# rbuler/multimodal-isic

Measured on AMD Instinct MI355X. Metric: bags/sec (train step) @ 64x224x224 patches/bag, higher is better.
Workload: dtype bf16; 1 GPU; ISIC-shaped attention-MIL: 256 bags x 64x224x224 patches + 128-d radiomics, ResNet-18 encoder, bf16 (BASELINE.json configs[1]); patches_per_bag=64, patch=3x224x224, radiomics_dim=128, parallelism=dp1

## Files before the change

### include/isic_hip.h

```cpp
#ifndef ISIC_HIP_H
#define ISIC_HIP_H

#include <stddef.h>
#include <stdint.h>

#ifdef __cplusplus
extern "C" {
#endif

#define ISIC_OK 0
#define ISIC_ERR_BAD_ARG (-1)
#define ISIC_ERR_UNSUPPORTED (-2)
#define ISIC_ERR_WORKSPACE (-3)
#define ISIC_ERR_LAUNCH (-4)

#define ISIC_ACT_NONE 0
#define ISIC_ACT_RELU 1
#define ISIC_ACT_TANH 2

int isic_abi_version(void);
const char* isic_target_arch(void);

int isic_gemm_f32(int transA, int transB, int M, int N, int K, const float* A, int lda, const float* B, int ldb,
                  float* C, int ldc, const float* bias, int act, float beta, void* stream);
// ... 231 lines not shown
                                   const float* rstd, int N, int H, int W, int C, int Ho, int Wo, const float* scale,
                                   const float* shift, double* dgamma, double* dbeta, void* stream);
int isic_bn_bwd_apply_pooled_bf16(const uint8_t* argmax, const uint16_t* dy_pooled, const uint16_t* x, const float* mean,
                                  const float* rstd, const float* gamma, const double* dgamma, const double* dbeta, int N,
                                  int H, int W, int C, int Ho, int Wo, const float* scale, const float* shift,
                                  uint16_t* dx, float* dgamma_f32, float* dbeta_f32, void* stream);
int isic_avgpool_fwd_bf16(const uint16_t* x, float* y, int N, int HW, int C, void* stream);
int isic_avgpool_bwd_bf16(const float* dy, uint16_t* dx, int N, int HW, int C, void* stream);
int isic_add_bf16(uint16_t* a, const uint16_t* b, int64_t n, void* stream);

int isic_gemm_f16(const uint16_t* A, const uint16_t* W, const float* bias, const uint16_t* residual, uint16_t* C,
                  int M, int N, int K, int act, int residual_rows, void* stream);
int isic_gemm_f16_stats(const uint16_t* A, const uint16_t* W, const float* bias, const uint16_t* residual, uint16_t* C,
                        float* row_stats, int M, int N, int K, int act, int residual_rows, void* stream);
int isic_gemm_f16_ln(const uint16_t* X, const uint16_t* Wg, const float* bias_b, const float* ln_c, const float* ln_stats,
                     int ln_parts, uint16_t* C, int M, int N, int K, int act, float eps, void* stream);
int isic_row_stats_f16(const uint16_t* x, float* stats, int64_t M, int N, float eps, void* stream);
int isic_vit_patchify_f16(const float* images_nchw, uint16_t* rows, int N, int C, int H, int W, int P, void* stream);
int isic_layernorm_f16(const uint16_t* x, const float* gamma, const float* beta, uint16_t* y, float* y_f32, int64_t M,
                       int N, float eps, void* stream);
int isic_attention_f16(const uint16_t* qkv, uint16_t* out, int n_images, int tokens, int heads, int head_dim,
                       void* stream);

#ifdef __cplusplus
}
#endif

#include "isic_hip_mxfp8.h"
#include "isic_hip_vit_train.h"
#include "isic_hip_convmae.h"
#include "isic_hip_convmae_train.h"
#include "isic_hip_mae.h"
#include "isic_hip_augment.h"

#endif
```

### multimodal-isic_amd/csrc/conv_wgrad.hip

```cpp
#include "common.h"

namespace {

struct WgradArgs {
  const unsigned short* x;
  const unsigned short* dy;
  float* dw;
  size_t split_stride;
  const int2* tab;
  int N, Hin, Win, Cin, Hout, Wout, Cout, Kh, Kw, stride, pad;
  int M;
  int ktiles;
  int ktiles_per_split;
  int co_tiles, ci_tiles;
};

__global__ void wgrad_table_kernel(int2* __restrict__ tab, int M, int Hout, int Wout, int Hin, int Win, int Cin,
                                   int stride, int pad) {
  const int m = blockIdx.x * blockDim.x + threadIdx.x;
  if (m >= M) return;
  const int hw = Hout * Wout;
  const int n = m / hw, r = m - n * hw;
  const int ho = r / Wout, wo = r - ho * Wout;
  int2 e;
// ... 168 lines not shown
  if (e < elems && g == 0) dw[e] += v;
}

struct WgradPlan {
  bool big;
  int tiles, splits, ktiles, ktiles_per_split;
  size_t table_bytes, partial_bytes, elems;
};

WgradPlan wgrad_plan(int N, int Cin, int Hout, int Wout, int Cout, int Kh, int Kw) {
  WgradPlan p;
  const int M = N * Hout * Wout;
  p.big = (Cin % 128 == 0) && (Cout % 128 == 0);
  const int tc = p.big ? 128 : 64, bkp = p.big ? 64 : 128;
  p.ktiles = ceil_div(M, bkp);
  p.tiles = (Cout / tc) * (Cin / tc) * Kh * Kw;
  int splits = ceil_div(1280, p.tiles);
  if (splits > ceil_div(p.ktiles, 8)) splits = ceil_div(p.ktiles, 8);
  if (splits < 1) splits = 1;
  if (splits > 4096) splits = 4096;
  p.ktiles_per_split = ceil_div(p.ktiles, splits);
  p.splits = ceil_div(p.ktiles, p.ktiles_per_split);
  p.table_bytes = ((size_t)M * sizeof(int2) + 255) / 256 * 256;
  p.elems = (size_t)Cout * Kh * Kw * Cin;
  p.partial_bytes = (size_t)p.splits * p.elems * sizeof(float);
  return p;
}

}

size_t isic_wgrad_c64_workspace_bytes(int N, int H, int W);
int isic_wgrad_c64_launch(const uint16_t* x, const uint16_t* dy, float* dw, int N, int H, int W, void* workspace,
                          hipStream_t stream);

size_t isic_wgrad_c128b_workspace_bytes(int N, int H, int W, int Cin, int Cout);
int isic_wgrad_c128b_launch(const uint16_t* x, const uint16_t* dy, float* dw, int N, int H, int W, int Cin, int Cout,
                            void* workspace, hipStream_t stream);

size_t isic_wgrad_s2_workspace_bytes(int N, int Hi, int Wi, int Cin, int Cout);
int isic_wgrad_s2_launch(const uint16_t* x, const uint16_t* dy, float* dw, int N, int Hi, int Wi, int Cin, int Cout,
                         void* workspace, hipStream_t stream);

namespace {
int conv2d_wgrad_dispatch(const uint16_t* x, const uint16_t* dy, float* dw, int N, int Hin, int Win, int Cin,
                          int Hout, int Wout, int Cout, int Kh, int Kw, int stride, int pad, void* workspace,
                          size_t workspace_bytes, int variant, void* stream);
}

extern "C" {

size_t isic_conv2d_wgrad_workspace_bytes(int N, int Cin, int Hout, int Wout, int Cout, int Kh, int Kw) {
  if (N <= 0 || Cin <= 0 || Hout <= 0 || Wout <= 0 || Cout <= 0 || Kh <= 0 || Kw <= 0) return 0;
  const WgradPlan p = wgrad_plan(N, Cin, Hout, Wout, Cout, Kh, Kw);
  size_t need = p.table_bytes + p.partial_bytes + 256;
  if (Cin == 64 && Cout == 64 && Kh == 3 && Kw == 3) {
    const size_t c64 = isic_wgrad_c64_workspace_bytes(N, Hout, Wout);
    if (c64 > need) need = c64;
  }
  if (Cin % 128 == 0 && Cout % 64 == 0 && Kh == 3 && Kw == 3) {
    const size_t c128b = isic_wgrad_c128b_workspace_bytes(N, Hout, Wout, Cin, Cout);
    if (c128b > need) need = c128b;
  }
  if (Cin % 64 == 0 && Cout % 128 == 0 && Kh == 3 && Kw == 3) {
    const size_t s2 = isic_wgrad_s2_workspace_bytes(N, 2 * Hout, 2 * Wout, Cin, Cout);
    if (s2 > need) need = s2;
  }
  return need;
}

int isic_conv2d_wgrad_bf16(const uint16_t* x, const uint16_t* dy, float* dw, int N, int Hin, int Win, int Cin,
                           int Hout, int Wout, int Cout, int Kh, int Kw, int stride, int pad, void* workspace,
                           size_t workspace_bytes, void* stream) {
  return conv2d_wgrad_dispatch(x, dy, dw, N, Hin, Win, Cin, Hout, Wout, Cout, Kh, Kw, stride, pad, workspace, workspace_bytes,
                               0, stream);
}

int isic_test_conv2d_wgrad_variant_bf16(const uint16_t* x, const uint16_t* dy, float* dw, int N, int Hin, int Win, int Cin,
                                        int Hout, int Wout, int Cout, int Kh, int Kw, int stride, int pad, void* workspace,
                                        size_t workspace_bytes, int variant, void* stream) {
  return conv2d_wgrad_dispatch(x, dy, dw, N, Hin, Win, Cin, Hout, Wout, Cout, Kh, Kw, stride, pad, workspace, workspace_bytes,
                               variant, stream);
}

}

namespace {

int conv2d_wgrad_dispatch(const uint16_t* x, const uint16_t* dy, float* dw, int N, int Hin, int Win, int Cin,
                          int Hout, int Wout, int Cout, int Kh, int Kw, int stride, int pad, void* workspace,
                          size_t workspace_bytes, int variant, void* stream) {
  ISIC_CHECK_ARG(x && dy && dw && workspace);
  ISIC_CHECK_ARG(N > 0 && Hin > 0 && Win > 0 && Hout > 0 && Wout > 0 && Kh > 0 && Kw > 0 && stride > 0 && pad >= 0);
  ISIC_CHECK_ARG((reinterpret_cast<uintptr_t>(workspace) & 255) == 0 && (reinterpret_cast<uintptr_t>(dw) & 15) == 0);
  ISIC_CHECK_ARG((variant & ~(16 | 32)) == 0);
  if (Cin % 64 != 0 || Cout % 64 != 0) return ISIC_ERR_UNSUPPORTED;
  const int64_t M64 = (int64_t)N * Hout * Wout;
  if (M64 > 0x7FFFFFFFLL / 2 || (int64_t)N * Hin * Win * Cin > 0x7FFFFFFFLL || Hout >= 32768 || Wout >= 32768)
    return ISIC_ERR_UNSUPPORTED;
  if (Cin == 64 && Cout == 64 && Kh == 3 && Kw == 3 && stride == 1 && pad == 1 && Hin == Hout && Win == Wout) {
    const size_t need = isic_wgrad_c64_workspace_bytes(N, Hin, Win);
    if (need != 0) {
      if (workspace_bytes < need) return ISIC_ERR_WORKSPACE;
      const int rc = isic_wgrad_c64_launch(x, dy, dw, N, Hin, Win, workspace, as_stream(stream));
      return rc != ISIC_OK ? rc : isic_launch_status();
    }
  }
  if (Cin % 128 == 0 && Cout % 64 == 0 && Kh == 3 && Kw == 3 && stride == 1 && pad == 1 && Hin == Hout && Win == Wout &&
// ... 46 lines not shown
```

### multimodal-isic_amd/csrc/conv_wgrad_c64.hip

```cpp

#include "common.h"

namespace {

constexpr int WT_H = 4, WT_W = 32;
constexpr int XP = 48;
constexpr int X_ROWS = WT_H + 2;
constexpr int X_BYTES = X_ROWS * XP * 128;
constexpr int DY_BYTES = WT_H * WT_W * 128;
constexpr int STAGE = X_BYTES + DY_BYTES;
constexpr int NSTAGE = 3;
constexpr int SCRATCH = NSTAGE * STAGE;
constexpr int LDS_TOTAL = SCRATCH + 1024;
constexpr int NDMA = 12;
constexpr int DW_ELEMS = 64 * 9 * 64;

struct WC64Args {
  const unsigned short* x;
  const unsigned short* dy;
  float* partial;
  int N, H, W, tiles_y, tiles_x, total_tiles, tiles_per_block;
};

__device__ __attribute__((aligned(256))) unsigned char g_wc64_zeros[2048];

__device__ __forceinline__ void glds16(const void* gsrc, unsigned lds_dst) {
  unsigned keep;
  asm volatile("s_mov_b32 %0, m0\n\ts_mov_b32 m0, %2\n\ts_nop 0\n\tglobal_load_lds_dwordx4 %1, off\n\ts_mov_b32 m0, %0"
               : "=&s"(keep) : "v"(gsrc), "s"(lds_dst) : "memory");
}

#ifdef WC64_STAMPS
__device__ unsigned long long g_wc64_stamps[256 * 64 * 4];
#define WC64_STAMP(kk, k) do { if (threadIdx.x == 512 && blockIdx.x < 256 && (kk) < 64) g_wc64_stamps[(blockIdx.x * 64 + (kk)) * 4 + (k)] = clock64(); } while (0)
#else
#define WC64_STAMP(kk, k) do { } while (0)
#endif

__global__ __launch_bounds__(768) void wgrad_c64_kernel(WC64Args a) {
  extern __shared__ __attribute__((aligned(16))) unsigned char smem[];
  typedef __attribute__((address_space(3))) s16x4* lds_s16x4;
  const unsigned lds0 = (unsigned)(size_t)(__attribute__((address_space(3))) unsigned char*)smem;
  const int tid = threadIdx.x, lane = tid & 63, wave12 = __builtin_amdgcn_readfirstlane(tid >> 6);
  const int t_begin = blockIdx.x * a.tiles_per_block;
  const int ntl = min(a.total_tiles - t_begin, a.tiles_per_block);

  if (wave12 >= 8) {
    const int p = wave12 - 8;
    const int tiles_img = a.tiles_y * a.tiles_x;
    struct Tile { int n, y0, x0; };
    auto advance = [&](Tile& tl) {
      tl.x0 += WT_W;
      if (tl.x0 >= a.W) {
        tl.x0 = 0; tl.y0 += WT_H;
        if (tl.y0 >= a.H) { tl.y0 = 0; tl.n += 1; }
      }
    };
    Tile ahead;
    {
      const int n = t_begin / tiles_img, rem = t_begin - n * tiles_img;
      const int ty = rem / a.tiles_x;
      ahead.n = n; ahead.y0 = ty * WT_H; ahead.x0 = (rem - ty * a.tiles_x) * WT_W;
    }
    const int r8 = lane >> 3, slot = lane & 7;
    const unsigned lane_e = (unsigned)(r8 * 128 + ((((slot >> 1) ^ ((r8 >> 1) & 1)) << 5) | ((slot & 1) << 4)));
    const unsigned lane_p = lane_e ^ (unsigned)((p & 1) << 6);
    const long long W128 = (long long)a.W * 128;
    const unsigned long long zeros = (unsigned long long)g_wc64_zeros;
    auto issue_tile = [&](const Tile& tl, int stage, bool live) {
      const long long org = ((long long)tl.n * a.H + tl.y0) * a.W + tl.x0;
      const unsigned long long xrow = (unsigned long long)a.x + (unsigned long long)((org - a.W - 1 + 8 * p) * 128);
      const unsigned long long yrow = (unsigned long long)a.dy + (unsigned long long)((org + 8 * p) * 128);
      const unsigned long long erow = (unsigned long long)a.x + (unsigned long long)((org + (long long)(2 * p - 1) * a.W + 31) * 128);
      const bool okx = (unsigned)(tl.x0 - 1 + 8 * p + r8) < (unsigned)a.W;
      const bool oky = (unsigned)(tl.x0 + 8 * p + r8) < (unsigned)a.W;
      const bool oke = (unsigned)(tl.x0 + 31 + r8) < (unsigned)a.W;
      const unsigned sbase = lds0 + (unsigned)stage * STAGE;
#pragma unroll
      for (int j = 0; j < NDMA; ++j) {
        unsigned long long rowaddr;
        bool okc, row_ok, real = live;
        unsigned lanev, dst;
        if (j < 6) {
          rowaddr = xrow + (unsigned long long)(j * W128);
          row_ok = (unsigned)(tl.y0 - 1 + j) < (unsigned)a.H; okc = okx; lanev = lane_p;
          dst = (unsigned)((j * XP + 8 * p) * 128);
        } else if (j < 10) {
          rowaddr = yrow + (unsigned long long)((j - 6) * W128);
          row_ok = (unsigned)(tl.y0 + j - 6) < (unsigned)a.H; okc = oky; lanev = lane_p;
          dst = (unsigned)(X_BYTES + ((j - 6) * 4 + p) * 1024);
        } else {
          const int pr = 2 * p + (j - 10);
          rowaddr = erow + (unsigned long long)((j - 10) * W128);
          row_ok = (unsigned)(tl.y0 - 1 + pr) < (unsigned)a.H; okc = oke; lanev = lane_e;
          real = real && pr < X_ROWS;
          dst = (unsigned)((pr * XP + 32) * 128);
        }
        const bool ok = okc && row_ok && real;
        const unsigned lo = ok ? (unsigned)rowaddr : (unsigned)zeros, hi = ok ? (unsigned)(rowaddr >> 32) : (unsigned)(zeros >> 32);
        const unsigned long long src = (((unsigned long long)hi << 32) | lo) + lanev;
        glds16(reinterpret_cast<const void*>(src), real ? sbase + dst : lds0 + SCRATCH);
      }
    };
    issue_tile(ahead, 0, true);
    advance(ahead);
    issue_tile(ahead, 1, ntl > 1);
    advance(ahead);
    for (int kk = 0; kk < ntl; ++kk) {
      WC64_STAMP(kk, 0);
      asm volatile("s_waitcnt vmcnt(%0)" ::"n"(NDMA) : "memory");
      WC64_STAMP(kk, 3);
      __builtin_amdgcn_s_barrier();
      WC64_STAMP(kk, 1);
      issue_tile(ahead, (kk + 2) % NSTAGE, kk + 2 < ntl);
      advance(ahead);
      WC64_STAMP(kk, 2);
    }
    return;
  }

  const int wave = wave12 & 3, half = wave12 >> 2;
  const int fg = lane >> 4, fi = lane & 15, fq = fi >> 2, fp = fi & 3;
  unsigned xaddr[3][2];
#pragma unroll
  for (int kw = 0; kw < 3; ++kw)
#pragma unroll
    for (int h = 0; h < 2; ++h) {
      const int px = 8 * fg + fq + kw + 4 * h;
      const int key = ((px >> 1) & 1) | (((px >> 3) & 1) << 1);
      xaddr[kw][h] = (unsigned)(px * 128 + ((wave ^ key) << 5) + fp * 8);
    }
  unsigned yaddr[2];
  {
    const int key = ((fq >> 1) & 1) | ((fg & 1) << 1);
#pragma unroll
    for (int c2 = 0; c2 < 2; ++c2) yaddr[c2] = (unsigned)(X_BYTES + (8 * fg + fq) * 128 + (((2 * half + c2) ^ key) << 5) + fp * 8);
// ... 73 lines not shown
    f32x4 t = red[0][q];
#pragma unroll
    for (int g = 1; g < 16; ++g) t += red[g][q];
    f32x4* out = reinterpret_cast<f32x4*>(dw) + e4;
    *out = *out + t;
  }
}

int wc64_blocks(int N, int H, int W, int* tiles_per_block) {
  const int cus = isic_cu_count();
  const int64_t total = (int64_t)N * ceil_div(H, WT_H) * ceil_div(W, WT_W);
  const int tpb = (int)ceil_div64(total, cus);
  if (tiles_per_block) *tiles_per_block = tpb;
  return (int)ceil_div64(total, tpb);
}

}

size_t isic_wgrad_c64_workspace_bytes(int N, int H, int W) {
  if ((int64_t)N * ceil_div(H, WT_H) * ceil_div(W, WT_W) > 0x7FFFFFFFLL) return 0;
  return (size_t)wc64_blocks(N, H, W, nullptr) * DW_ELEMS * sizeof(float);
}

int isic_wgrad_c64_launch(const uint16_t* x, const uint16_t* dy, float* dw, int N, int H, int W, void* workspace,
                          hipStream_t stream) {
  WC64Args a;
  a.x = x; a.dy = dy; a.partial = reinterpret_cast<float*>(workspace);
  a.N = N; a.H = H; a.W = W;
  a.tiles_y = ceil_div(H, WT_H); a.tiles_x = ceil_div(W, WT_W);
  a.total_tiles = N * a.tiles_y * a.tiles_x;
  const int grid = wc64_blocks(N, H, W, &a.tiles_per_block);
  static IsicPerDeviceOnce once;
  if (isic_once_per_device(once, [] {
        return hipFuncSetAttribute(reinterpret_cast<const void*>(wgrad_c64_kernel), hipFuncAttributeMaxDynamicSharedMemorySize,
                                  LDS_TOTAL);
      }) != hipSuccess)
    return ISIC_ERR_LAUNCH;
  hipLaunchKernelGGL(wgrad_c64_kernel, dim3(grid), dim3(768), LDS_TOTAL, stream, a);
  hipLaunchKernelGGL(wgrad_c64_reduce_kernel, dim3(DW_ELEMS / 64), dim3(256), 0, stream, a.partial, dw, grid);
  return ISIC_OK;
}
```

### multimodal-isic_amd/isic_hip/build.py

```python
from __future__ import annotations

import os
import shutil
import subprocess
import sys
from concurrent.futures import ThreadPoolExecutor

HERE = os.path.dirname(os.path.abspath(__file__))
PKG = os.path.dirname(HERE)
CSRC = os.path.join(PKG, "csrc")
OBJ = os.path.join(CSRC, "build")
LIB = os.path.join(HERE, "libisic_hip.so")
ARCH = "gfx950"
FLAGS = ["-O3", "-fPIC", "-std=c++17", f"--offload-arch={ARCH}", "-Wall", "-Wno-unused-function",
         "-Wno-unused-variable"]


def _hipcc():
    for c in (os.environ.get("HIPCC"), shutil.which("hipcc"), "/opt/rocm/bin/hipcc"):
        if c and os.path.exists(c):
            return c
    raise RuntimeError("hipcc not found: libisic_hip.so cannot be built")


def sources():
    return sorted(os.path.join(CSRC, f) for f in os.listdir(CSRC) if f.endswith(".hip"))


def _stale(target, deps):
    if not os.path.exists(target):
        return True
    t = os.path.getmtime(target)
    return any(os.path.getmtime(d) > t for d in deps)


def build(force=False, verbose=True, jobs=None):
    hipcc = _hipcc()
    os.makedirs(OBJ, exist_ok=True)
    headers = [os.path.join(CSRC, f) for f in os.listdir(CSRC) if f.endswith(".h")]
    headers += [os.path.join(os.path.dirname(PKG), "include", h)
                for h in ("isic_hip.h", "isic_hip_mxfp8.h", "isic_hip_vit_train.h", "isic_hip_convmae.h",
                          "isic_hip_convmae_train.h", "isic_hip_mae.h", "isic_hip_augment.h")]
    todo, objs = [], []
    for src in sources():
        obj = os.path.join(OBJ, os.path.basename(src)[:-4] + ".o")
        objs.append(obj)
        if force or _stale(obj, [src] + headers):
            todo.append((src, obj))

    def compile_one(so):
        src, obj = so
        cmd = [hipcc] + FLAGS + ["-c", src, "-o", obj]
        r = subprocess.run(cmd, capture_output=True, text=True)
        if r.returncode != 0:
            raise RuntimeError(f"hipcc failed for {src}:\n{r.stdout}\n{r.stderr}")
        if verbose and r.stderr.strip():
            sys.stderr.write(r.stderr)
        return obj

    if todo:
        if verbose:
            print(f"[isic_hip] compiling {len(todo)} HIP source(s) for {ARCH}", flush=True)
        with ThreadPoolExecutor(max_workers=jobs or min(8, os.cpu_count() or 4)) as ex:
            list(ex.map(compile_one, todo))
    if force or todo or _stale(LIB, objs):
        cmd = [hipcc, "-shared", "-fPIC", f"--offload-arch={ARCH}", "-o", LIB] + objs
        r = subprocess.run(cmd, capture_output=True, text=True)
        if r.returncode != 0:
            raise RuntimeError(f"link failed:\n{r.stdout}\n{r.stderr}")
        if verbose:
            print(f"[isic_hip] linked {LIB}", flush=True)
    return LIB


if __name__ == "__main__":
# ... 2 lines not shown
```

### multimodal-isic_amd/isic_hip/encoder.py

```python
from __future__ import annotations

import os

import torch
import torch.nn as nn

from .lib import ERR_UNSUPPORTED, IsicHipError, call

LAYERS = ((64, 1), (128, 2), (256, 2), (512, 2))
BN_EPS, BN_MOMENTUM = 1e-5, 0.1
STAT_SLOTS = 256
STEM_STAT_SLOTS = 1024
_BF16 = torch.bfloat16


def _empty(shape, like, dtype=_BF16):
    return torch.empty(shape, device=like.device, dtype=dtype)


class _ConvSpec:
    __slots__ = ("name", "cin", "cout", "k", "stride", "pad")

    def __init__(self, name, cin, cout, k, stride, pad):
        self.name, self.cin, self.cout, self.k, self.stride, self.pad = name, cin, cout, k, stride, pad
# ... 21 lines not shown
            self._register(name + ".bias", nn.Parameter(torch.zeros(c)))
            self._register(name + ".running_mean", torch.zeros(c), buffer=True)
            self._register(name + ".running_var", torch.ones(c), buffer=True)
            self._register(name + ".num_batches_tracked", torch.zeros((), dtype=torch.long), buffer=True)

        conv("conv1", in_ch, 64, 7, 2, 3)
        bn("bn1", 64)
        inp = 64
        self.blocks = []
        for li, (planes, stride) in enumerate(self.layers_cfg, start=1):
            for b in range(2):
                pre = f"layer{li}.{b}"
                st = stride if b == 0 else 1
                conv(f"{pre}.conv1", inp, planes, 3, st, 1)
                bn(f"{pre}.bn1", planes)
                conv(f"{pre}.conv2", planes, planes, 3, 1, 1)
                bn(f"{pre}.bn2", planes)
                ds = st != 1 or inp != planes
                if ds:
                    conv(f"{pre}.downsample.0", inp, planes, 1, st, 0)
                    bn(f"{pre}.downsample.1", planes)
                self.blocks.append((pre, ds))
                inp = planes
        self._wcache = {}
        self._wgrad_ws = None
        self._zeros = None
        self._zeros_used = 0
        self._side = None
        self.wgrad_stream = False
        self.fuse_bn_backward = False
        self.mask_identity_gradient = True
        self.pair_downsample_gradient = True
        self.fold_shortcut_norm = True
        self._tape_fused = False
        self.grad_ready_hook = None

    def _register(self, dotted, tensor, buffer=False):
        parts = dotted.split(".")
        mod = self
        for p in parts[:-1]:
            if not hasattr(mod, p):
                mod.add_module(p, nn.Module())
            mod = getattr(mod, p)
        if buffer:
            mod.register_buffer(parts[-1], tensor)
        else:
            mod.register_parameter(parts[-1], tensor)

    def _get(self, dotted):
        mod = self
        for p in dotted.split("."):
            mod = getattr(mod, p)
        return mod

    def _apply(self, fn, *a, **k):
        out = super()._apply(fn, *a, **k)
        for name in self.specs:
            p = self._get(name + ".weight")
            if not p.data.is_contiguous(memory_format=torch.channels_last):
                p.data = p.data.contiguous(memory_format=torch.channels_last)
        self._wcache = {}
        return out

    def prepare_weights(self):
        for name, sp in self.specs.items():
            p = self._get(name + ".weight")
            if not p.is_cuda:
# ... 191 lines not shown
                call("isic_bn_stats_bf16", c, rows, C, acc[0], acc[1])
            mean = torch.empty(C, device=dev, dtype=torch.float32)
            rstd = torch.empty(C, device=dev, dtype=torch.float32)
            call("isic_bn_finalize", acc[0], acc[1], slots, rows, C, gamma.data, beta.data, BN_EPS, BN_MOMENTUM, scale,
                 shift, mean, rstd, self._get(name + ".running_mean"), self._get(name + ".running_var"))
        else:
            call("isic_bn_eval_affine", gamma.data, beta.data, self._get(name + ".running_mean"),
                 self._get(name + ".running_var"), BN_EPS, C, scale, shift)
        return mean, rstd, scale, shift

    def _bn_bwd(self, dy, c, y, st, name, relu, want_residual, mask_from_x=False):
        mean, rstd, scale, shift = st[:4]
        mask = st[4] if len(st) > 4 else None
        N, H, W, C = c.shape
        rows = N * H * W
        gamma, beta = self._get(name + ".weight"), self._get(name + ".bias")
        acc = self._zeros64((2, C), c.device)
        if mask is not None and relu and not mask_from_x:
            call("isic_bn_bwd_reduce_mask_bf16", dy, c, mask, mean, rstd, rows, C, acc[0], acc[1])
            dx = _empty(c.shape, c)
            dres = _empty(c.shape, c) if want_residual else None
            call("isic_bn_bwd_apply_mask_bf16", dy, c, mask, mean, rstd, gamma.data, acc[0], acc[1], rows, C, dx, dres,
                 self._grad_buffer(gamma), self._grad_buffer(beta))
            return dx, dres
        sc, sh = (scale, shift) if (mask_from_x and relu) else (None, None)
        yy = None if (mask_from_x or not relu) else y
        call("isic_bn_bwd_reduce_bf16", dy, c, yy, mean, rstd, rows, C, int(relu), sc, sh, acc[0], acc[1])
        dx = _empty(c.shape, c)
        dres = _empty(c.shape, c) if want_residual else None
        call("isic_bn_bwd_apply_bf16", dy, c, yy, mean, rstd, gamma.data, acc[0], acc[1], rows, C, int(relu), sc, sh, dx,
             dres, self._grad_buffer(gamma), self._grad_buffer(beta))
        return dx, dres

    def _fire(self, names):
        if self.grad_ready_hook is not None:
            dev = self._get("conv1.weight").device
            self._on_side(dev, (), lambda: self.grad_ready_hook(names))

    def pack_input(self, images):
        if images.dim() != 4 or images.shape[1] != self.in_ch:
            raise ValueError(f"expected images[N,{self.in_ch},H,W], got {tuple(images.shape)}")
        if not images.is_cuda:
            raise IsicHipError("ResNet18Encoder runs on the MI355X only (no CPU fallback)")
        if images.dtype not in (torch.float32, _BF16):
            images = images.float()
        images = images.contiguous()
        N, C, H, W = images.shape
        out = torch.empty((N, H, W, 4), device=images.device, dtype=_BF16)
        call("isic_nchw_to_nhwc4_bf16", images, int(images.dtype == _BF16), out, N, C, H, W)
        return out

    def block_forward(self, x, pre, ds):
        idn, cd, std, idn_affine = x, None, None, None
        if ds:
            cd, accd = self._conv_fwd(x, f"{pre}.downsample.0")
            if self.training and self.fold_shortcut_norm:
                std = self._bn_affine(cd, f"{pre}.downsample.1", accd)
                idn, idn_affine = cd, (std[2], std[3])
            else:
                idn, std = self._bn_fwd(cd, f"{pre}.downsample.1", False, acc=accd)
        c1, acc1 = self._conv_fwd(x, f"{pre}.conv1")
        a1, st1 = self._bn_fwd(c1, f"{pre}.bn1", True, acc=acc1)
        c2, acc2 = self._conv_fwd(a1, f"{pre}.conv2")
        out, st2 = self._bn_fwd(c2, f"{pre}.bn2", True, residual=idn, acc=acc2, residual_affine=idn_affine)
        return out, (x, c1, a1, st1, c2, out, st2, cd, std)

    def block_backward(self, g, pre, ds, saved):
        dx, names, _ = self.block_backward_fused(g, pre, ds, saved)
        return dx, names

    def block_backward_fused(self, g, pre, ds, saved, g_sums=None, prev=None):
        x, c1, a1, st1, c2, out, st2, cd, std = saved
        masked_join = (self.mask_identity_gradient and not ds and g_sums is None and len(st2) > 4 and
                       not (prev is not None and len(prev[6]) > 4 and self._dgrad_bnbwd_ok(c1.shape, f"{pre}.conv1", tuple(x.shape)))
                       and self._maskadd_ok(c1.shape, f"{pre}.conv1", tuple(x.shape)))
        if g_sums is not None:
            dc2, dres = self._bn_bwd_from_sums(g, c2, st2, f"{pre}.bn2", g_sums), g
        else:
            dc2, dres = self._bn_bwd(g, c2, out, st2, f"{pre}.bn2", True, not masked_join)
        self._conv_wgrad(a1, dc2, f"{pre}.conv2")
        if len(st1) > 4 and self._dgrad_bnbwd_ok(dc2.shape, f"{pre}.conv2", tuple(a1.shape)):
            dz1, sums1 = self._conv_dgrad_bnbwd(dc2, f"{pre}.conv2", tuple(a1.shape), st1[4], c1)
            del dc2
            dc1 = self._bn_bwd_from_sums(dz1, c1, st1, f"{pre}.bn1", sums1)
            del dz1
        else:
            da1 = self._conv_dgrad(dc2, f"{pre}.conv2", tuple(a1.shape))
            del dc2
            dc1, _ = self._bn_bwd(da1, c1, a1, st1, f"{pre}.bn1", True, False, mask_from_x=True)
            del da1
        self._conv_wgrad(x, dc1, f"{pre}.conv1")
        names = [f"{pre}.conv2.weight", f"{pre}.bn2.weight", f"{pre}.bn2.bias", f"{pre}.conv1.weight",
                 f"{pre}.bn1.weight", f"{pre}.bn1.bias"]
        dx_sums = None
        if ds:
            dcd, _ = self._bn_bwd(dres, cd, None, std, f"{pre}.downsample.1", False, False)
            self._conv_wgrad(x, dcd, f"{pre}.downsample.0")
            dx = self._conv_dgrad_pair(dc1, f"{pre}.conv1", dcd, f"{pre}.downsample.0", tuple(x.shape))
            names += [f"{pre}.downsample.0.weight", f"{pre}.downsample.1.weight", f"{pre}.downsample.1.bias"]
        elif prev is not None and len(prev[6]) > 4 and self._dgrad_bnbwd_ok(dc1.shape, f"{pre}.conv1", tuple(x.shape)):
            dx, dx_sums = self._conv_dgrad_bnbwd(dc1, f"{pre}.conv1", tuple(x.shape), prev[6][4], prev[4], addend=dres)
        elif masked_join:
            dx = self._conv_dgrad(dc1, f"{pre}.conv1", tuple(x.shape), addend=g, addend_mask=st2[4])
        else:
            dx = self._conv_dgrad(dc1, f"{pre}.conv1", tuple(x.shape), addend=dres)
        return dx, names, dx_sums

    def run_forward(self, images, save):
        self.prepare_weights()
        x0 = self.pack_input(images)
        self._arena_reset(x0.device)
        N, H, W, _ = x0.shape
        Ho, Wo = (H + 6 - 7) // 2 + 1, (W + 6 - 7) // 2 + 1
        ws, _ = self._weights("conv1", False)
        c = _empty((N, Ho, Wo, 64), x0)
        acc0 = None
        if self.training:
            acc0 = self._zeros64((2, STEM_STAT_SLOTS, 64), x0.device)
            call("isic_conv_stem_fwd_stats_bf16", x0, ws, c, N, H, W, Ho, Wo, acc0[0], acc0[1], STEM_STAT_SLOTS)
        else:
            call("isic_conv_stem_fwd_bf16", x0, ws, c, N, H, W, Ho, Wo)
        st0 = self._bn_affine(c, "bn1", acc0)
        Hp, Wp = (Ho + 2 - 3) // 2 + 1, (Wo + 2 - 3) // 2 + 1
        p = _empty((N, Hp, Wp, 64), c)
        am = torch.empty((N, Hp, Wp, 64), device=c.device, dtype=torch.uint8) if save else None
        csel = _empty((N, Hp, Wp, 64), c) if save else None
        call("isic_bn_relu_maxpool3x3s2_fwd_sel_bf16", c, st0[2], st0[3], p, am, csel, N, Ho, Wo, 64, Hp, Wp)
        tape = {"x0": x0, "stem": (c, st0, am, csel, (N, Ho, Wo, 64)), "blocks": [],
                "fused_bn_backward": bool(self.fuse_bn_backward)} if save else None
        x = p
        for pre, ds in self.blocks:
            x, saved = self.block_forward(x, pre, ds)
            if save:
                tape["blocks"].append(saved)
        N, Hf, Wf, Cf = x.shape
        feat = torch.empty((N, Cf), device=x.device, dtype=torch.float32)
        call("isic_avgpool_fwd_bf16", x, feat, N, Hf * Wf, Cf)
        if save:
            tape["final_shape"] = (N, Hf, Wf, Cf)
            if self.training:
                for name in self._bn_names():
                    self._get(name + ".num_batches_tracked").add_(1)
        return feat, tape

    @torch.no_grad()
    def run_tokens(self, images, stage=3):
        if self.training:
            raise IsicHipError("run_tokens is an inference path: call eval() first (running BatchNorm statistics)")
        self.prepare_weights()
        x0 = self.pack_input(images)
        self._arena_reset(x0.device)
        N, H, W, _ = x0.shape
        Ho, Wo = (H + 6 - 7) // 2 + 1, (W + 6 - 7) // 2 + 1
        ws, _ = self._weights("conv1", False)
        c = _empty((N, Ho, Wo, 64), x0)
        call("isic_conv_stem_fwd_bf16", x0, ws, c, N, H, W, Ho, Wo)
        st0 = self._bn_affine(c, "bn1", None)
        Hp, Wp = (Ho + 2 - 3) // 2 + 1, (Wo + 2 - 3) // 2 + 1
        x = _empty((N, Hp, Wp, 64), c)
        call("isic_bn_relu_maxpool3x3s2_fwd_bf16", c, st0[2], st0[3], x, None, N, Ho, Wo, 64, Hp, Wp)
        for pre, ds in self.blocks[:2 * int(stage)]:
            x, _ = self.block_forward(x, pre, ds)
        N, Hf, Wf, Cf = x.shape
        return x.float().view(N, Hf * Wf, Cf)

    def _bn_names(self):
        names = ["bn1"]
        for pre, ds in self.blocks:
            names += [f"{pre}.bn1", f"{pre}.bn2"] + ([f"{pre}.downsample.1"] if ds else [])
        return names

    def run_backward(self, tape, dfeat):
        if not self.training:
            raise IsicHipError("encoder backward needs train() mode (batch-statistics BatchNorm)")
        N, Hf, Wf, Cf = tape["final_shape"]
        self._tape_fused = bool(tape.get("fused_bn_backward", False))
        self._arena_reset(dfeat.device)
        g = torch.empty((N, Hf, Wf, Cf), device=dfeat.device, dtype=_BF16)
        call("isic_avgpool_bwd_bf16", dfeat.float().contiguous(), g, N, Hf * Wf, Cf)
        g_sums = None
        for bi in range(len(self.blocks) - 1, -1, -1):
            pre, ds = self.blocks[bi]
            prev = tape["blocks"][bi - 1] if bi > 0 else None
            g, names, g_sums = self.block_backward_fused(g, pre, ds, tape["blocks"][bi], g_sums=g_sums, prev=prev)
            self._fire(names)
        c, st0, am, csel, yshape = tape["stem"]
        N, Ho, Wo, _ = yshape
        _, Hp, Wp, _ = g.shape
        mean, rstd, scale, shift = st0
        gamma, beta = self._get("bn1.weight"), self._get("bn1.bias")
        acc = self._zeros64((2, 64), c.device)
        call("isic_bn_bwd_reduce_bf16", g, csel, None, mean, rstd, N * Hp * Wp, 64, 1, scale, shift, acc[0], acc[1])
        x0 = tape["x0"]
        p = self._get("conv1.weight")
        gw, gg, gb = self._grad_buffer(p), self._grad_buffer(gamma), self._grad_buffer(beta)
        ws = self._workspace(call("isic_conv_stem_wgrad_workspace_bytes"), c.device)
        self._on_side(c.device, (x0, c, g, am, acc),
                      lambda: call("isic_conv_stem_wgrad_bn_pooled_bf16", x0, c, am, g, mean, rstd, gamma.data, scale, shift,
                                   acc[0], acc[1], gw, gg, gb, N, x0.shape[1], x0.shape[2], Ho, Wo, Hp, Wp, ws, ws.numel()))
        self._fire(["conv1.weight", "bn1.weight", "bn1.bias"])
        if self._side is not None:
            torch.cuda.current_stream(c.device).wait_stream(self._side)

    def forward(self, images):
        if torch.is_grad_enabled() and self.training:
            return _EncoderFn.apply(images, self, *[p for p in self.parameters()])
        feat, _ = self.run_forward(images, save=False)
        return feat

# ... 16 lines not shown
```

### multimodal-isic_amd/isic_hip/lib.py

```python
from __future__ import annotations

import ctypes
import os
import re

import torch

HERE = os.path.dirname(os.path.abspath(__file__))
PKG = os.path.dirname(HERE)
LIB_PATH = os.path.join(HERE, "libisic_hip.so")
_HEADER_CANDIDATES = (
    os.path.join(os.path.dirname(PKG), "include", "isic_hip.h"),
    os.path.join(PKG, "include", "isic_hip.h"),
)

ERRORS = {0: "ISIC_OK", -1: "ISIC_ERR_BAD_ARG", -2: "ISIC_ERR_UNSUPPORTED", -3: "ISIC_ERR_WORKSPACE",
          -4: "ISIC_ERR_LAUNCH"}

_SCALARS = {
    "int": ctypes.c_int, "int32_t": ctypes.c_int32, "int64_t": ctypes.c_int64, "uint32_t": ctypes.c_uint32,
    "uint64_t": ctypes.c_uint64, "size_t": ctypes.c_size_t, "float": ctypes.c_float, "double": ctypes.c_double,
}


class IsicHipError(RuntimeError):

    def __init__(self, msg, code=None):
        super().__init__(msg)
        self.code = code


ERR_UNSUPPORTED = -2


def header_path():
    for p in _HEADER_CANDIDATES:
        if os.path.exists(p):
            return p
    raise IsicHipError("include/isic_hip.h not found next to the package")


def extension_header_paths():
    inc = os.path.dirname(header_path())
    return [os.path.join(inc, h) for h in ("isic_hip_mxfp8.h", "isic_hip_vit_train.h", "isic_hip_convmae.h",
                                                      "isic_hip_convmae_train.h", "isic_hip_mae.h", "isic_hip_augment.h")]


def test_header_path():
    return os.path.join(os.path.dirname(header_path()), "isic_hip_test.h")


def parse_header(path=None):
    text = open(path or header_path()).read()
    text = re.sub(r"/\*.*?\*/", " ", text, flags=re.S)
    text = re.sub(r"//[^\n]*", " ", text)
    protos = {}
    for m in re.finditer(r"\b(int|size_t|const\s+char\s*\*)\s+(isic_\w+)\s*\(([^)]*)\)\s*;", text):
        ret, name, params = m.group(1), m.group(2), m.group(3)
        restype = ctypes.c_char_p if "char" in ret else _SCALARS[ret]
        args = []
        for prm in (p.strip() for p in params.split(",")):
            if not prm or prm == "void":
                continue
            is_ptr = "*" in prm
            toks = prm.replace("*", " * ").split()
            pname = toks[-1]
            base = [t for t in toks[:-1] if t not in ("const", "*")]
            if is_ptr:
                args.append((ctypes.c_void_p, pname, True))
            else:
                args.append((_SCALARS[base[-1]], pname, False))
        protos[name] = (restype, args)
    return protos


class _Lib:
    def __init__(self):
        if not os.path.exists(LIB_PATH):
# ... 71 lines not shown
```

Measured before the change: 927.0 bags/s.

## Fuse BatchNorm backward apply into the C64 3x3 weight-gradient kernel

Adds a templated mode of the 64-channel 3x3 wgrad kernel that loads dy, the pre-BN activation and the ReLU mask or scale/shift directly. It computes the BN-backward input gradient dc in registers, writes it to global memory and feeds the same values into LDS as the dy operand. The encoder's basic-block backward uses this path for conv2/bn2 and conv1/bn1 when shapes match, replacing a separate BN-backward apply kernel and the wgrad kernel's re-read of dc. In exchange the kernel uses more registers and issues more global loads, and the fused path is skipped when a separate wgrad stream is in use.

```diff
diff --git a/include/isic_hip.h b/include/isic_hip.h
--- a/include/isic_hip.h
+++ b/include/isic_hip.h
@@ -287,5 +287,6 @@
 #include "isic_hip_convmae_train.h"
 #include "isic_hip_mae.h"
 #include "isic_hip_augment.h"
+#include "isic_hip_wgrad_bnbwd.h"
 
 #endif
diff --git a/include/isic_hip_wgrad_bnbwd.h b/include/isic_hip_wgrad_bnbwd.h
--- /dev/null
+++ b/include/isic_hip_wgrad_bnbwd.h
@@ -0,0 +1,22 @@
+#ifndef ISIC_HIP_WGRAD_BNBWD_H
+#define ISIC_HIP_WGRAD_BNBWD_H
+
+#include <stddef.h>
+#include <stdint.h>
+
+#ifdef __cplusplus
+extern "C" {
+#endif
+
+size_t isic_conv2d_wgrad_bnbwd_supported(int N, int H, int W, int Cin, int Cout, int Kh, int Kw, int stride, int pad,
+                                         int has_mask);
+int isic_conv2d_wgrad_bnbwd_bf16(const uint16_t* x, const uint16_t* dz, const uint16_t* c, const uint8_t* relu_mask,
+                                 const float* mean, const float* rstd, const float* gamma, const double* sum_dz,
+                                 const double* sum_dzx, const float* scale, const float* shift, uint16_t* dc, float* dw,
+                                 float* dgamma_f32, float* dbeta_f32, int N, int H, int W, void* workspace,
+                                 size_t workspace_bytes, void* stream);
+
+#ifdef __cplusplus
+}
+#endif
+#endif
diff --git a/multimodal-isic_amd/csrc/conv_wgrad.hip b/multimodal-isic_amd/csrc/conv_wgrad.hip
--- a/multimodal-isic_amd/csrc/conv_wgrad.hip
+++ b/multimodal-isic_amd/csrc/conv_wgrad.hip
@@ -224,6 +224,11 @@
 size_t isic_wgrad_c64_workspace_bytes(int N, int H, int W);
 int isic_wgrad_c64_launch(const uint16_t* x, const uint16_t* dy, float* dw, int N, int H, int W, void* workspace,
                           hipStream_t stream);
+int isic_wgrad_c64_bnbwd_launch(const uint16_t* x, const uint16_t* g, const uint16_t* c, const uint8_t* relu_mask,
+                                const float* mean, const float* rstd, const float* gamma, const double* dgamma,
+                                const double* dbeta, const float* scale, const float* shift, uint16_t* dc, float* dw,
+                                float* dgamma_f32, float* dbeta_f32, int N, int H, int W, void* workspace,
+                                hipStream_t stream);
 
 size_t isic_wgrad_c128b_workspace_bytes(int N, int H, int W, int Cin, int Cout);
 int isic_wgrad_c128b_launch(const uint16_t* x, const uint16_t* dy, float* dw, int N, int H, int W, int Cin, int Cout,
@@ -265,6 +270,34 @@
                            size_t workspace_bytes, void* stream) {
   return conv2d_wgrad_dispatch(x, dy, dw, N, Hin, Win, Cin, Hout, Wout, Cout, Kh, Kw, stride, pad, workspace, workspace_bytes,
                                0, stream);
+}
+
+size_t isic_conv2d_wgrad_bnbwd_supported(int N, int H, int W, int Cin, int Cout, int Kh, int Kw, int stride, int pad,
+                                         int has_mask) {
+  (void)has_mask;
+  if (N <= 0 || H <= 0 || W <= 0 || Cin != 64 || Cout != 64 || Kh != 3 || Kw != 3 || stride != 1 || pad != 1) return 0;
+  if ((int64_t)N * H * W * 64 > 0x7FFFFFFFLL || H >= 32768 || W >= 32768) return 0;
+  return isic_wgrad_c64_workspace_bytes(N, H, W) != 0 ? 1 : 0;
+}
+
+int isic_conv2d_wgrad_bnbwd_bf16(const uint16_t* x, const uint16_t* dz, const uint16_t* c, const uint8_t* relu_mask,
+                                 const float* mean, const float* rstd, const float* gamma, const double* sum_dz,
+                                 const double* sum_dzx, const float* scale, const float* shift, uint16_t* dc, float* dw,
+                                 float* dgamma_f32, float* dbeta_f32, int N, int H, int W, void* workspace,
+                                 size_t workspace_bytes, void* stream) {
+  ISIC_CHECK_ARG(x && dz && c && mean && rstd && gamma && sum_dz && sum_dzx && dc && dw && workspace);
+  ISIC_CHECK_ARG(N > 0 && H > 0 && W > 0);
+  ISIC_CHECK_ARG((scale == nullptr) == (shift == nullptr));
+  ISIC_CHECK_ARG((dgamma_f32 == nullptr) == (dbeta_f32 == nullptr));
+  ISIC_CHECK_ARG((reinterpret_cast<uintptr_t>(workspace) & 255) == 0 && (reinterpret_cast<uintptr_t>(dw) & 15) == 0);
+  ISIC_CHECK_ARG(((reinterpret_cast<uintptr_t>(x) | reinterpret_cast<uintptr_t>(dz) | reinterpret_cast<uintptr_t>(c) |
+                   reinterpret_cast<uintptr_t>(dc)) & 15) == 0);
+  if (!relu_mask && !scale) return ISIC_ERR_UNSUPPORTED;
+  if (!isic_conv2d_wgrad_bnbwd_supported(N, H, W, 64, 64, 3, 3, 1, 1, relu_mask != nullptr)) return ISIC_ERR_UNSUPPORTED;
+  if (workspace_bytes < isic_wgrad_c64_workspace_bytes(N, H, W)) return ISIC_ERR_WORKSPACE;
+  const int rc = isic_wgrad_c64_bnbwd_launch(x, dz, c, relu_mask, mean, rstd, gamma, sum_dzx, sum_dz, scale, shift, dc, dw,
+                                             dgamma_f32, dbeta_f32, N, H, W, workspace, as_stream(stream));
+  return rc != ISIC_OK ? rc : isic_launch_status();
 }
 
 int isic_test_conv2d_wgrad_variant_bf16(const uint16_t* x, const uint16_t* dy, float* dw, int N, int Hin, int Win, int Cin,
diff --git a/multimodal-isic_amd/csrc/conv_wgrad_c64.hip b/multimodal-isic_amd/csrc/conv_wgrad_c64.hip
--- a/multimodal-isic_amd/csrc/conv_wgrad_c64.hip
+++ b/multimodal-isic_amd/csrc/conv_wgrad_c64.hip
@@ -1,5 +1,6 @@
 
 #include "common.h"
+#include "pool_grad.h"
 
 namespace {
 
@@ -22,6 +23,15 @@
   int N, H, W, tiles_y, tiles_x, total_tiles, tiles_per_block;
 };
 
+struct WC64BnArgs : WC64Args {
+  const unsigned short* c;
+  const unsigned char* mask;
+  const float *mean, *rstd, *gamma, *scale, *shift;
+  const double *dgamma, *dbeta;
+  unsigned short* dc;
+  float *dgamma_f32, *dbeta_f32;
+};
+
 __device__ __attribute__((aligned(256))) unsigned char g_wc64_zeros[2048];
 
 __device__ __forceinline__ void glds16(const void* gsrc, unsigned lds_dst) {
@@ -29,6 +39,33 @@
   asm volatile("s_mov_b32 %0, m0\n\ts_mov_b32 m0, %2\n\ts_nop 0\n\tglobal_load_lds_dwordx4 %1, off\n\ts_mov_b32 m0, %0"
                : "=&s"(keep) : "v"(gsrc), "s"(lds_dst) : "memory");
 }
+
+__device__ __forceinline__ u32x4 wc64_load16(const void* gsrc) {
+  u32x4 v;
+  asm volatile("global_load_dwordx4 %0, %1, off" : "=v"(v) : "v"(gsrc) : "memory");
+  return v;
+}
+__device__ __forceinline__ unsigned wc64_load1(const void* gsrc) {
+  unsigned v;
+  asm volatile("global_load_ubyte %0, %1, off" : "=v"(v) : "v"(gsrc) : "memory");
+  return v;
+}
+template <int N>
+__device__ __forceinline__ void wc64_landed(u32x4 (&g)[4], u32x4 (&c)[4]) {
+  asm volatile("s_waitcnt vmcnt(%8)"
+               : "+v"(g[0]), "+v"(g[1]), "+v"(g[2]), "+v"(g[3]), "+v"(c[0]), "+v"(c[1]), "+v"(c[2]), "+v"(c[3])
+               : "n"(N) : "memory");
+}
+template <int N>
+__device__ __forceinline__ void wc64_landed(u32x4 (&g)[4], u32x4 (&c)[4], unsigned (&m)[4]) {
+  asm volatile("s_waitcnt vmcnt(%12)"
+               : "+v"(g[0]), "+v"(g[1]), "+v"(g[2]), "+v"(g[3]), "+v"(c[0]), "+v"(c[1]), "+v"(c[2]), "+v"(c[3]),
+                 "+v"(m[0]), "+v"(m[1]), "+v"(m[2]), "+v"(m[3])
+               : "n"(N) : "memory");
+}
+template <int V> struct WC64Int { static constexpr int value = V; };
+template <int MODE> struct WC64Mode { typedef WC64BnArgs Args; };
+template <> struct WC64Mode<0> { typedef WC64Args Args; };
 
 #ifdef WC64_STAMPS
 __device__ unsigned long long g_wc64_stamps[256 * 64 * 4];
@@ -37,7 +74,8 @@
 #define WC64_STAMP(kk, k) do { } while (0)
 #endif
 
-__global__ __launch_bounds__(768) void wgrad_c64_kernel(WC64Args a) {
+template <int MODE>
+__global__ __launch_bounds__(768) void wgrad_c64_kernel(typename WC64Mode<MODE>::Args a) {
   extern __shared__ __attribute__((aligned(16))) unsigned char smem[];
   typedef __attribute__((address_space(3))) s16x4* lds_s16x4;
   const unsigned lds0 = (unsigned)(size_t)(__attribute__((address_space(3))) unsigned char*)smem;
@@ -86,6 +124,7 @@
           row_ok = (unsigned)(tl.y0 - 1 + j) < (unsigned)a.H; okc = okx; lanev = lane_p;
           dst = (unsigned)((j * XP + 8 * p) * 128);
         } else if (j < 10) {
+          if constexpr (MODE != 0) continue;
           rowaddr = yrow + (unsigned long long)((j - 6) * W128);
           row_ok = (unsigned)(tl.y0 + j - 6) < (unsigned)a.H; okc = oky; lanev = lane_p;
           dst = (unsigned)(X_BYTES + ((j - 6) * 4 + p) * 1024);
@@ -102,6 +141,107 @@
         glds16(reinterpret_cast<const void*>(src), real ? sbase + dst : lds0 + SCRATCH);
       }
     };
+    if constexpr (MODE != 0) {
+      constexpr int NLD = MODE == 3 ? 12 : 8;
+      const int cg = (int)((lane_p & 127u) >> 4);
+      float kA[8], kB[8], kD[8], sc[8], sh[8];
+      {
+        const float inv_rows = 1.f / (float)((int64_t)a.N * a.H * a.W);
+        if (blockIdx.x == 0 && p == 0 && a.dgamma_f32) {
+          a.dgamma_f32[lane] += (float)a.dgamma[lane];
+          a.dbeta_f32[lane] += (float)a.dbeta[lane];
+        }
+#pragma unroll
+        for (int j = 0; j < 8; ++j) {
+#pragma clang fp contract(off)
+          const int c = cg * 8 + j;
+          const float mu = a.mean[c], rs = a.rstd[c], k1 = a.gamma[c] * rs;
+          const float k2 = (float)a.dbeta[c] * inv_rows, k3 = (float)a.dgamma[c] * inv_rows;
+          kA[j] = k1; kB[j] = -k1 * k3 * rs; kD[j] = k1 * __builtin_fmaf(k3 * rs, mu, -k2);
+          sc[j] = MODE == 2 ? a.scale[c] : 0.f; sh[j] = MODE == 2 ? a.shift[c] : 0.f;
+        }
+#pragma unroll
+        for (int j = 0; j < 8; ++j) asm volatile("" : "+v"(kA[j]), "+v"(kB[j]), "+v"(kD[j]), "+v"(sc[j]), "+v"(sh[j]));
+      }
+      u32x4 rg[2][4], rc[2][4];
+      unsigned rm[2][4];
+      auto dy_off = [&](const Tile& tl, int j, bool& ok) -> long long {
+        ok = (unsigned)(tl.x0 + 8 * p + r8) < (unsigned)a.W && (unsigned)(tl.y0 + j) < (unsigned)a.H;
+        return ((((long long)tl.n * a.H + tl.y0 + j) * a.W + tl.x0 + 8 * p) << 7) + (long long)lane_p;
+      };
+      auto load_dy = [&](const Tile& tl, bool live, auto SET) {
+        constexpr int S = decltype(SET)::value;
+#pragma unroll
+        for (int j = 0; j < WT_H; ++j) {
+          bool ok;
+          const long long off = dy_off(tl, j, ok);
+          ok = ok && live;
+          const unsigned char* zp = g_wc64_zeros + lane_p;
+          rg[S][j] = wc64_load16(ok ? reinterpret_cast<const unsigned char*>(a.dy) + off : zp);
+          rc[S][j] = wc64_load16(ok ? reinterpret_cast<const unsigned char*>(a.c) + off : zp);
+          if constexpr (MODE == 3) rm[S][j] = wc64_load1(ok ? a.mask + (off >> 4) : zp);
+        }
+      };
+      auto commit_dy = [&](const Tile& tl, int stage, auto SET) {
+        constexpr int S = decltype(SET)::value;
+        if constexpr (MODE == 3) wc64_landed<8 + NLD>(rg[S], rc[S], rm[S]);
+        else wc64_landed<8 + NLD>(rg[S], rc[S]);
+        const unsigned sdy = lds0 + (unsigned)stage * STAGE + (unsigned)(X_BYTES + p * 1024 + lane * 16);
+#pragma unroll
+        for (int j = 0; j < WT_H; ++j) {
+          bool ok;
+          const long long off = dy_off(tl, j, ok);
+          float g[8], xv[8], yv[8], o[8];
+          isic_pool::unpack8(rg[S][j], g);
+          isic_pool::unpack8(rc[S][j], xv);
+          if constexpr (MODE == 2) {
+#pragma unroll
+            for (int e = 0; e < 8; ++e) yv[e] = __builtin_fmaf(xv[e], sc[e], sh[e]);
+          } else {
+            const unsigned m = rm[S][j];
+#pragma unroll
+            for (int e = 0; e < 8; ++e) yv[e] = ((m >> e) & 1u) ? 1.f : 0.f;
+          }
+#pragma unroll
+          for (int e = 0; e < 8; ++e) {
+            const float dz = !(yv[e] > 0.f) ? 0.f : g[e];
+            o[e] = __builtin_fmaf(kA[e], dz, __builtin_fmaf(kB[e], xv[e], kD[e]));
+          }
+          u32x4 v = isic_pool::pack8(o);
+          if (!ok) v = (u32x4){0u, 0u, 0u, 0u};
+          *(__attribute__((address_space(3))) u32x4*)(size_t)(sdy + (unsigned)(j * 4 * 1024)) = v;
+          if (ok) __builtin_nontemporal_store(v, reinterpret_cast<u32x4*>(reinterpret_cast<unsigned char*>(a.dc) + off));
+        }
+      };
+      Tile next = ahead;
+      issue_tile(ahead, 0, true);
+      load_dy(ahead, true, WC64Int<0>());
+      advance(ahead);
+      issue_tile(ahead, 1, ntl > 1);
+      load_dy(ahead, ntl > 1, WC64Int<1>());
+      advance(ahead);
+      commit_dy(next, 0, WC64Int<0>());
+      advance(next);
+      auto step = [&](int kk, auto SET) {
+        constexpr int S = decltype(SET)::value;
+        asm volatile("s_waitcnt lgkmcnt(0)" ::: "memory");
+        __builtin_amdgcn_s_barrier();
+        issue_tile(ahead, (kk + 2) % NSTAGE, kk + 2 < ntl);
+        load_dy(ahead, kk + 2 < ntl, WC64Int<S>());
+        advance(ahead);
+        if (kk + 1 < ntl) {
+          commit_dy(next, (kk + 1) % NSTAGE, WC64Int<S ^ 1>());
+          advance(next);
+        }
+      };
+      for (int kk = 0; kk < ntl; kk += 2) {
+        step(kk, WC64Int<0>());
+        if (kk + 1 >= ntl) break;
+        step(kk + 1, WC64Int<1>());
+      }
+      asm volatile("s_waitcnt vmcnt(0)" ::: "memory");
+      return;
+    }
     issue_tile(ahead, 0, true);
     advance(ahead);
     issue_tile(ahead, 1, ntl > 1);
@@ -241,11 +381,38 @@
   const int grid = wc64_blocks(N, H, W, &a.tiles_per_block);
   static IsicPerDeviceOnce once;
   if (isic_once_per_device(once, [] {
-        return hipFuncSetAttribute(reinterpret_cast<const void*>(wgrad_c64_kernel), hipFuncAttributeMaxDynamicSharedMemorySize,
+        return hipFuncSetAttribute(reinterpret_cast<const void*>(wgrad_c64_kernel<0>), hipFuncAttributeMaxDynamicSharedMemorySize,
                                   LDS_TOTAL);
       }) != hipSuccess)
     return ISIC_ERR_LAUNCH;
-  hipLaunchKernelGGL(wgrad_c64_kernel, dim3(grid), dim3(768), LDS_TOTAL, stream, a);
+  hipLaunchKernelGGL(wgrad_c64_kernel<0>, dim3(grid), dim3(768), LDS_TOTAL, stream, a);
   hipLaunchKernelGGL(wgrad_c64_reduce_kernel, dim3(DW_ELEMS / 64), dim3(256), 0, stream, a.partial, dw, grid);
   return ISIC_OK;
 }
+
+int isic_wgrad_c64_bnbwd_launch(const uint16_t* x, const uint16_t* g, const uint16_t* c, const uint8_t* relu_mask,
+                                const float* mean, const float* rstd, const float* gamma, const double* dgamma,
+                                const double* dbeta, const float* scale, const float* shift, uint16_t* dc, float* dw,
+                                float* dgamma_f32, float* dbeta_f32, int N, int H, int W, void* workspace,
+                                hipStream_t stream) {
+  WC64BnArgs a;
+  a.x = x; a.dy = g; a.partial = reinterpret_cast<float*>(workspace);
+  a.N = N; a.H = H; a.W = W;
+  a.tiles_y = ceil_div(H, WT_H); a.tiles_x = ceil_div(W, WT_W);
+  a.total_tiles = N * a.tiles_y * a.tiles_x;
+  a.c = c; a.mask = relu_mask; a.mean = mean; a.rstd = rstd; a.gamma = gamma; a.scale = scale; a.shift = shift;
+  a.dgamma = dgamma; a.dbeta = dbeta; a.dc = dc; a.dgamma_f32 = dgamma_f32; a.dbeta_f32 = dbeta_f32;
+  const int grid = wc64_blocks(N, H, W, &a.tiles_per_block);
+  static IsicPerDeviceOnce once[2];
+  const int m = relu_mask ? 1 : 0;
+  if (isic_once_per_device(once[m], [m] {
+        return hipFuncSetAttribute(m ? reinterpret_cast<const void*>(wgrad_c64_kernel<3>)
+                                     : reinterpret_cast<const void*>(wgrad_c64_kernel<2>),
+                                   hipFuncAttributeMaxDynamicSharedMemorySize, LDS_TOTAL);
+      }) != hipSuccess)
+    return ISIC_ERR_LAUNCH;
+  if (m) hipLaunchKernelGGL(wgrad_c64_kernel<3>, dim3(grid), dim3(768), LDS_TOTAL, stream, a);
+  else hipLaunchKernelGGL(wgrad_c64_kernel<2>, dim3(grid), dim3(768), LDS_TOTAL, stream, a);
+  hipLaunchKernelGGL(wgrad_c64_reduce_kernel, dim3(DW_ELEMS / 64), dim3(256), 0, stream, a.partial, dw, grid);
+  return ISIC_OK;
+}
diff --git a/multimodal-isic_amd/isic_hip/build.py b/multimodal-isic_amd/isic_hip/build.py
--- a/multimodal-isic_amd/isic_hip/build.py
+++ b/multimodal-isic_amd/isic_hip/build.py
@@ -40,7 +40,7 @@
     headers = [os.path.join(CSRC, f) for f in os.listdir(CSRC) if f.endswith(".h")]
     headers += [os.path.join(os.path.dirname(PKG), "include", h)
                 for h in ("isic_hip.h", "isic_hip_mxfp8.h", "isic_hip_vit_train.h", "isic_hip_convmae.h",
-                          "isic_hip_convmae_train.h", "isic_hip_mae.h", "isic_hip_augment.h")]
+                          "isic_hip_convmae_train.h", "isic_hip_mae.h", "isic_hip_augment.h", "isic_hip_wgrad_bnbwd.h")]
     todo, objs = [], []
     for src in sources():
         obj = os.path.join(OBJ, os.path.basename(src)[:-4] + ".o")
diff --git a/multimodal-isic_amd/isic_hip/encoder.py b/multimodal-isic_amd/isic_hip/encoder.py
--- a/multimodal-isic_amd/isic_hip/encoder.py
+++ b/multimodal-isic_amd/isic_hip/encoder.py
@@ -77,7 +77,9 @@
         self.mask_identity_gradient = True
         self.pair_downsample_gradient = True
         self.fold_shortcut_norm = True
+        self.fuse_bn_apply_wgrad = True
         self._tape_fused = False
+        self._tape_apply_wgrad = False
         self.grad_ready_hook = None
 
     def _register(self, dotted, tensor, buffer=False):
@@ -335,6 +337,36 @@
              dres, self._grad_buffer(gamma), self._grad_buffer(beta))
         return dx, dres
 
+    def _bn_bwd_wgrad(self, dy, c, st, name, x, conv, mask_from_x=False):
+        if not self._tape_apply_wgrad or self.wgrad_stream:
+            return None
+        mean, rstd, scale, shift = st[:4]
+        mask = st[4] if (len(st) > 4 and not mask_from_x) else None
+        if mask is None and not mask_from_x:
+            return None
+        sp = self.specs[conv]
+        N, H, W, C = c.shape
+        if tuple(x.shape) != tuple(c.shape) or not call("isic_conv2d_wgrad_bnbwd_supported", N, H, W, sp.cin, sp.cout, sp.k,
+                                                        sp.k, sp.stride, sp.pad, int(mask is not None)):
+            return None
+        p = self._get(conv + ".weight")
+        gw = self._grad_buffer(p)
+        if not gw.is_contiguous(memory_format=torch.channels_last):
+            raise IsicHipError(f"{conv}.weight.grad must be channels_last ([O][Kh][Kw][I] memory)")
+        gamma, beta = self._get(name + ".weight"), self._get(name + ".bias")
+        rows = N * H * W
+        acc = self._zeros64((2, C), c.device)
+        if mask is not None:
+            call("isic_bn_bwd_reduce_mask_bf16", dy, c, mask, mean, rstd, rows, C, acc[0], acc[1])
+            scale = shift = None
+        else:
+            call("isic_bn_bwd_reduce_bf16", dy, c, None, mean, rstd, rows, C, 1, scale, shift, acc[0], acc[1])
+        dc = _empty(c.shape, c)
+        ws = self._workspace(call("isic_conv2d_wgrad_workspace_bytes", N, C, H, W, C, sp.k, sp.k), c.device)
+        call("isic_conv2d_wgrad_bnbwd_bf16", x, dy, c, mask, mean, rstd, gamma.data, acc[1], acc[0], scale, shift, dc, gw,
+             self._grad_buffer(gamma), self._grad_buffer(beta), N, H, W, ws, ws.numel())
+        return dc
+
     def _fire(self, names):
         if self.grad_ready_hook is not None:
             dev = self._get("conv1.weight").device
@@ -379,20 +411,27 @@
                        and self._maskadd_ok(c1.shape, f"{pre}.conv1", tuple(x.shape)))
         if g_sums is not None:
             dc2, dres = self._bn_bwd_from_sums(g, c2, st2, f"{pre}.bn2", g_sums), g
-        else:
-            dc2, dres = self._bn_bwd(g, c2, out, st2, f"{pre}.bn2", True, not masked_join)
-        self._conv_wgrad(a1, dc2, f"{pre}.conv2")
+            self._conv_wgrad(a1, dc2, f"{pre}.conv2")
+        else:
+            dc2 = self._bn_bwd_wgrad(g, c2, st2, f"{pre}.bn2", a1, f"{pre}.conv2") if masked_join else None
+            dres = None
+            if dc2 is None:
+                dc2, dres = self._bn_bwd(g, c2, out, st2, f"{pre}.bn2", True, not masked_join)
+                self._conv_wgrad(a1, dc2, f"{pre}.conv2")
         if len(st1) > 4 and self._dgrad_bnbwd_ok(dc2.shape, f"{pre}.conv2", tuple(a1.shape)):
             dz1, sums1 = self._conv_dgrad_bnbwd(dc2, f"{pre}.conv2", tuple(a1.shape), st1[4], c1)
             del dc2
             dc1 = self._bn_bwd_from_sums(dz1, c1, st1, f"{pre}.bn1", sums1)
             del dz1
+            self._conv_wgrad(x, dc1, f"{pre}.conv1")
         else:
             da1 = self._conv_dgrad(dc2, f"{pre}.conv2", tuple(a1.shape))
             del dc2
-            dc1, _ = self._bn_bwd(da1, c1, a1, st1, f"{pre}.bn1", True, False, mask_from_x=True)
+            dc1 = self._bn_bwd_wgrad(da1, c1, st1, f"{pre}.bn1", x, f"{pre}.conv1", mask_from_x=True)
+            if dc1 is None:
+                dc1, _ = self._bn_bwd(da1, c1, a1, st1, f"{pre}.bn1", True, False, mask_from_x=True)
+                self._conv_wgrad(x, dc1, f"{pre}.conv1")
             del da1
-        self._conv_wgrad(x, dc1, f"{pre}.conv1")
         names = [f"{pre}.conv2.weight", f"{pre}.bn2.weight", f"{pre}.bn2.bias", f"{pre}.conv1.weight",
                  f"{pre}.bn1.weight", f"{pre}.bn1.bias"]
         dx_sums = None
@@ -430,7 +469,8 @@
         csel = _empty((N, Hp, Wp, 64), c) if save else None
         call("isic_bn_relu_maxpool3x3s2_fwd_sel_bf16", c, st0[2], st0[3], p, am, csel, N, Ho, Wo, 64, Hp, Wp)
         tape = {"x0": x0, "stem": (c, st0, am, csel, (N, Ho, Wo, 64)), "blocks": [],
-                "fused_bn_backward": bool(self.fuse_bn_backward)} if save else None
+                "fused_bn_backward": bool(self.fuse_bn_backward),
+                "fused_bn_apply_wgrad": bool(self.fuse_bn_apply_wgrad)} if save else None
         x = p
         for pre, ds in self.blocks:
             x, saved = self.block_forward(x, pre, ds)
@@ -478,6 +518,7 @@
             raise IsicHipError("encoder backward needs train() mode (batch-statistics BatchNorm)")
         N, Hf, Wf, Cf = tape["final_shape"]
         self._tape_fused = bool(tape.get("fused_bn_backward", False))
+        self._tape_apply_wgrad = bool(tape.get("fused_bn_apply_wgrad", False))
         self._arena_reset(dfeat.device)
         g = torch.empty((N, Hf, Wf, Cf), device=dfeat.device, dtype=_BF16)
         call("isic_avgpool_bwd_bf16", dfeat.float().contiguous(), g, N, Hf * Wf, Cf)
diff --git a/multimodal-isic_amd/isic_hip/lib.py b/multimodal-isic_amd/isic_hip/lib.py
--- a/multimodal-isic_amd/isic_hip/lib.py
+++ b/multimodal-isic_amd/isic_hip/lib.py
@@ -43,7 +43,7 @@
 def extension_header_paths():
     inc = os.path.dirname(header_path())
     return [os.path.join(inc, h) for h in ("isic_hip_mxfp8.h", "isic_hip_vit_train.h", "isic_hip_convmae.h",
-                                                      "isic_hip_convmae_train.h", "isic_hip_mae.h", "isic_hip_augment.h")]
+                                                      "isic_hip_convmae_train.h", "isic_hip_mae.h", "isic_hip_augment.h", "isic_hip_wgrad_bnbwd.h")]
 
 
 def test_header_path():
```

Result: faster. 937.1 bags/s (median of 6 runs) (+1.1%).
